# OrangeSodahub/ORV

Measured on AMD Instinct MI355X. Metric: denoise-steps/sec, higher is better.
Workload: dtype bf16; 1 GPU; configs[1]: CogVideoX-2B singleview 320x480x17f (latents [B,5,32,40,60], S=3226), DDIM 50-step schedule, guidance 1.0, trajectory-conditioned; batch_per_gpu=4, num_layers=30, parallelism=replica x1 (no collective), valid=True

## Files before the change

orv_amd/csrc/gemm_d8.hip:

```cpp
#include "gemm_common.hpp"
#include <type_traits>

namespace {
using namespace orv_gemm;

__device__ __forceinline__ void d8_unpack8(const uint4 u, float (&f)[8]) {
    f[0] = bf2f(u.x & 0xffff); f[1] = bf2f(u.x >> 16); f[2] = bf2f(u.y & 0xffff); f[3] = bf2f(u.y >> 16);
    f[4] = bf2f(u.z & 0xffff); f[5] = bf2f(u.z >> 16); f[6] = bf2f(u.w & 0xffff); f[7] = bf2f(u.w >> 16);
}
__device__ __forceinline__ uint4 d8_pack8(const float (&f)[8]) {
    return make_uint4(pack2bf(f[0], f[1]), pack2bf(f[2], f[3]), pack2bf(f[4], f[5]), pack2bf(f[6], f[7]));
}
__device__ __forceinline__ float d8_sum_quad(float v) {
    v += __uint_as_float(__builtin_amdgcn_update_dpp(0, __float_as_uint(v), 0xB1, 0xF, 0xF, true));
    v += __uint_as_float(__builtin_amdgcn_update_dpp(0, __float_as_uint(v), 0x4E, 0xF, 0xF, true));
    return v;
}
__device__ __forceinline__ float d8_shl4(float v) {
    return __uint_as_float(__builtin_amdgcn_update_dpp(0, __float_as_uint(v), 0x104, 0xF, 0xF, true));
}
__device__ __forceinline__ float d8_shr4(float v) {
    return __uint_as_float(__builtin_amdgcn_update_dpp(0, __float_as_uint(v), 0x114, 0xF, 0xF, true));
}
__device__ __forceinline__ unsigned long long d8_uniform64(unsigned long long u) {
    const unsigned lo = __builtin_amdgcn_readfirstlane((unsigned)u), hi = __builtin_amdgcn_readfirstlane((unsigned)(u >> 32));
    return ((unsigned long long)hi << 32) | lo;
}

__device__ __forceinline__ void d8_glds_v(const void* gsrc, const char* lds_dst) {
    const unsigned d = __builtin_amdgcn_readfirstlane((unsigned)(uintptr_t)(const __attribute__((address_space(3))) char*)lds_dst);
    asm volatile("s_mov_b32 m0, %1\n\ts_nop 0\n\tglobal_load_lds_dwordx4 %0, off" :: "v"(gsrc), "s"(d) : "memory", "m0");
}
__device__ __forceinline__ void d8_issue_rows(const GemmArgs& p, const int row0, const int colg, const int lane, const char* slab) {
#pragma unroll
    for (int j = 0; j < 4; ++j) {
        const int mc = min(row0 + 8 * j + (lane >> 3), p.M - 1);
        long rr = mc;
        if (p.r_mod > 0) rr = mc % p.r_mod;
        else if (p.c_rows > 0) rr = (long)(mc / p.c_rows) * p.c_bstride + p.c_off + mc % p.c_rows;
        d8_glds_v(p.R + rr * p.ldr + colg + 8 * (lane & 7), slab + j * 1024);
    }
}
template <int BN, int EPI>
constexpr bool d8_rlds() {
#ifdef ORV_D8_RLDS
    return BN <= 192 && (EPI == 2 || EPI == 3);
#else
    return false;
#endif
}

template <int BN, int EPI, int RB = 2>
__device__ __forceinline__ void d8_epilogue(const GemmArgs& p, f32x4 (&acc)[RB][BN / 16], const int row0, const int col0, const int lane,
                                            char* const scr, const char* const rslab = nullptr) {
    constexpr int NG = BN / 64;
    constexpr bool RLDS = d8_rlds<BN, EPI>();
    const int g = lane >> 4, r16 = lane & 15;
    const int c = lane & 7, rr8 = lane >> 3;
    int woff[4];
#pragma unroll
    for (int blk = 0; blk < 4; ++blk) {
        const int L = 8 * (blk >> 1) + 2 * g + (blk & 1);
        woff[blk] = r16 * 256 + ((L ^ (r16 & 7)) << 4);
    }
    const int roff0 = rr8 * 256 + (((2 * c) ^ rr8) << 4), roff1 = rr8 * 256 + (((2 * c + 1) ^ rr8) << 4);

    constexpr bool GATH = EPI == 2 || EPI == 3;
    using row_t = std::conditional_t<GATH && BN == 256, int, long>;
    row_t orow[RB][2];
    bool valid[RB][2];
#pragma unroll
    for (int rb = 0; rb < RB; ++rb)
#pragma unroll
        for (int j = 0; j < 2; ++j) {
            const int m = row0 + rb * 16 + 8 * j + rr8;
            valid[rb][j] = m < p.M;
            const int mc = min(m, p.M - 1);
            orow[rb][j] = mc;
            if (p.c_rows > 0) orow[rb][j] = (row_t)((long)(mc / p.c_rows) * p.c_bstride + p.c_off + mc % p.c_rows);
        }
    const float *gate_a = nullptr, *gate_b = nullptr;
    int gseg = 0;
    bool in_a[RB][2];
#pragma unroll
    for (int rb = 0; rb < RB; ++rb) in_a[rb][0] = in_a[rb][1] = true;
    if (EPI == 2 && p.gate) {
        const int mf = __builtin_amdgcn_readfirstlane(row0);
        long of = min(mf, p.M - 1), ol = min(mf + 16 * RB - 1, p.M - 1);
        if (p.c_rows > 0) {
            of = (long)(of / p.c_rows) * p.c_bstride + p.c_off + of % p.c_rows;
            ol = (long)(ol / p.c_rows) * p.c_bstride + p.c_off + ol % p.c_rows;
        }
        const int bf_ = (int)(of / p.seq), bl_ = (int)(ol / p.seq);
        const int gf_ = orv_group_of((int)(of % p.seq), p.n_text, p.per_group);
        const int gl_ = orv_group_of((int)(ol % p.seq), p.n_text, p.per_group);
        gate_a = p.gate + bf_ * p.gate_b + gf_ * p.gate_g;
        gseg = 1;
        if (bf_ != bl_ || gf_ != gl_) {
            gate_b = p.gate + bl_ * p.gate_b + gl_ * p.gate_g;
            const int ea_ = gf_ == 0 ? p.n_text : (p.per_group > 0 ? p.n_text + gf_ * p.per_group : p.seq);
            const long end_a = (long)bf_ * p.seq + min(ea_, p.seq);
            const long start_b = (long)bl_ * p.seq + (gl_ == 0 ? 0 : p.n_text + (gl_ - 1) * max(p.per_group, 0));
            bool other = false;
#pragma unroll
            for (int rb = 0; rb < RB; ++rb)
#pragma unroll
                for (int j = 0; j < 2; ++j) {
                    in_a[rb][j] = orow[rb][j] < end_a;
                    other = other || !(in_a[rb][j] || orow[rb][j] >= start_b);
                }
            gseg = (BN == 256 || __builtin_amdgcn_ballot_w64(other) != 0) ? 3 : 2;
        }
    }
    uint4 r8[RB][2];
    auto load_row = [&](int cg, int rb, int j) {
        long rr = orow[rb][j];
        if (p.r_mod > 0) rr = min(row0 + rb * 16 + 8 * j + rr8, p.M - 1) % p.r_mod;
        return *(const uint4*)(p.R + rr * p.ldr + col0 + 64 * cg + 8 * c);
    };
    auto take_rows = [&](int cg, uint4 (&dst)[RB][2]) {
        asm volatile("s_waitcnt vmcnt(0)" ::: "memory");
        __builtin_amdgcn_sched_barrier(0);
#pragma unroll
        for (int rb = 0; rb < RB; ++rb)
#pragma unroll
            for (int j = 0; j < 2; ++j) dst[rb][j] = *(const uint4*)(rslab + (rb * 16 + 8 * j + rr8) * 128 + c * 16);
        if (cg + 1 < NG) {
            asm volatile("s_waitcnt lgkmcnt(0)" ::: "memory");
            __builtin_amdgcn_sched_barrier(0);
            d8_issue_rows(p, row0, col0 + 64 * (cg + 1), lane, rslab);
        }
    };
    if (RLDS) {
        take_rows(0, r8);
    } else if (GATH) {
#pragma unroll
        for (int rb = 0; rb < RB; ++rb)
#pragma unroll
            for (int j = 0; j < 2; ++j) r8[rb][j] = load_row(0, rb, j);
    }
    const int bp = c << 5;
    uint32_t bsrc[NG];
    float gsrc_a[NG], gsrc_b[NG];
#pragma unroll
    for (int cg = 0; cg < NG; ++cg) { bsrc[cg] = 0; gsrc_a[cg] = gsrc_b[cg] = 1.f; }
    if constexpr (GATH) {
        if (p.bias) {
#pragma unroll
            for (int cg = 0; cg < NG; ++cg) bsrc[cg] = p.bias[col0 + 64 * cg + lane];
        }
        if (gseg == 1 || gseg == 2) {
#pragma unroll
            for (int cg = 0; cg < NG; ++cg) gsrc_a[cg] = gate_a[col0 + 64 * cg + lane];
        }
        if (gseg == 2) {
#pragma unroll
            for (int cg = 0; cg < NG; ++cg) gsrc_b[cg] = gate_b[col0 + 64 * cg + lane];
        }
    }
    auto spread8 = [&](uint32_t src, uint32_t (&o)[8]) {
        asm volatile("ds_bpermute_b32 %0, %8, %9\n\tds_bpermute_b32 %1, %8, %9 offset:4\n\tds_bpermute_b32 %2, %8, %9 offset:8\n\t"
                     "ds_bpermute_b32 %3, %8, %9 offset:12\n\tds_bpermute_b32 %4, %8, %9 offset:16\n\tds_bpermute_b32 %5, %8, %9 offset:20\n\t"
                     "ds_bpermute_b32 %6, %8, %9 offset:24\n\tds_bpermute_b32 %7, %8, %9 offset:28\n\ts_waitcnt lgkmcnt(0)"
                     : "=&v"(o[0]), "=&v"(o[1]), "=&v"(o[2]), "=&v"(o[3]), "=&v"(o[4]), "=&v"(o[5]), "=&v"(o[6]), "=&v"(o[7])
                     : "v"(bp), "v"(src));
    };

#pragma unroll
    for (int cg = 0; cg < NG; ++cg) {
        const int col8 = col0 + 64 * cg + 8 * c;
        if (RLDS && cg > 0) take_rows(cg, r8);
        float b8[8];
#pragma unroll
        for (int e = 0; e < 8; ++e) b8[e] = 0.f;
        if (p.bias) {
            if constexpr (GATH) {
                uint32_t o[8];
                spread8(bsrc[cg], o);
#pragma unroll
                for (int e = 0; e < 8; ++e) b8[e] = bf2f((bf16_t)o[e]);
            } else {
                d8_unpack8(*(const uint4*)(p.bias + col8), b8);
            }
        }
        float ga[8], be[8];
        int region = 2;
        float post = 1.f;
        if constexpr (EPI == 4) {
            region = __builtin_amdgcn_readfirstlane((col0 + 64 * cg) / (p.qn_heads * 64));
            const bf16_t* gam = region == 0 ? p.qn_gq : p.qn_gk;
            const bf16_t* bet = region == 0 ? p.qn_bq : p.qn_bk;
            post = region == 0 ? p.qn_premul : 1.f;
#pragma unroll
            for (int e = 0; e < 8; ++e) { ga[e] = 1.f; be[e] = 0.f; }
            if (region < 2 && gam) d8_unpack8(*(const uint4*)(gam + 8 * c), ga);
            if (region < 2 && bet) d8_unpack8(*(const uint4*)(bet + 8 * c), be);
        }
        float g8[8];
#pragma unroll
        for (int e = 0; e < 8; ++e) g8[e] = 1.f;
        if (gseg == 1 || gseg == 2) {
            uint32_t o[8];
            spread8(__float_as_uint(gsrc_a[cg]), o);
#pragma unroll
            for (int e = 0; e < 8; ++e) g8[e] = __uint_as_float(o[e]);
        }

#pragma unroll
        for (int rb = 0; rb < RB; ++rb) {
#pragma unroll
            for (int blk = 0; blk < 4; ++blk) *(f32x4*)(scr + woff[blk]) = acc[rb][4 * cg + blk];
            float v[2][8];
            auto read_v = [&](int j) {
                const f32x4 lo = *(const f32x4*)(scr + j * 2048 + roff0), hi = *(const f32x4*)(scr + j * 2048 + roff1);
                v[j][0] = lo[0]; v[j][1] = lo[1]; v[j][2] = lo[2]; v[j][3] = lo[3];
                v[j][4] = hi[0]; v[j][5] = hi[1]; v[j][6] = hi[2]; v[j][7] = hi[3];
            };
            if constexpr (!GATH) { read_v(0); read_v(1); }
#pragma unroll
            for (int j = 0; j < 2; ++j) {
                if constexpr (GATH) {
                    asm volatile("" ::: "memory");
                    read_v(j);
                }
                float (&w)[8] = v[j];
                uint4 rcur;
                if constexpr (GATH) {
                    rcur = r8[rb][j];
                    if (!RLDS && cg + 1 < NG) r8[rb][j] = load_row(cg + 1, rb, j);
                }
#pragma unroll
                for (int e = 0; e < 8; ++e) w[e] += b8[e];
                bf16_t* crow = p.C + orow[rb][j] * p.ldc + col8;
                if (p.Y && valid[rb][j]) *(uint4*)(p.Y + orow[rb][j] * p.ldy + col8) = d8_pack8(w);
                if constexpr (EPI == 4) {
                    if (region < 2) {
                        float hi[8];
#pragma unroll
                        for (int e = 0; e < 8; ++e) hi[e] = d8_shl4(w[e]);
                        float s = 0.f;
#pragma unroll
                        for (int e = 0; e < 8; ++e) s += w[e];
#pragma unroll
                        for (int e = 0; e < 8; ++e) s += hi[e];
                        s = d8_sum_quad(s);
                        const float s_up = d8_shr4(s);
                        const float mean = (c < 4 ? s : s_up) * (1.f / 64.f);
                        float sq = 0.f;
#pragma unroll
                        for (int e = 0; e < 8; ++e) { w[e] -= mean; sq = qkln_sq(w[e], sq); }
#pragma unroll
                        for (int e = 0; e < 8; ++e) { hi[e] -= mean; sq = qkln_sq(hi[e], sq); }
                        sq = d8_sum_quad(sq);
                        const float sq_up = d8_shr4(sq);
                        const float rstd = rsqrtf((c < 4 ? sq : sq_up) * (1.f / 64.f) + p.qn_eps);
#pragma unroll
                        for (int e = 0; e < 8; ++e) w[e] = qkln_affine(w[e], rstd, ga[e], be[e], post);
                    }
                }
                if (EPI == 1) {
#pragma unroll
                    for (int e = 0; e < 8; ++e) w[e] = gelu_tanh(w[e]);
                }
                if (EPI == 2) {
                    float rv[8], gg[8];
                    d8_unpack8(rcur, rv);
#pragma unroll
                    for (int e = 0; e < 8; ++e) gg[e] = g8[e];
                    if (gseg == 2) {
                        uint32_t o[8];
                        spread8(__float_as_uint(gsrc_b[cg]), o);
#pragma unroll
                        for (int e = 0; e < 8; ++e) gg[e] = in_a[rb][j] ? g8[e] : __uint_as_float(o[e]);
                    }
                    if (gseg == 3 && j == 0) {
                        f32x4 q[2][2];
#pragma unroll
                        for (int jj = 0; jj < 2; ++jj) {
                            const unsigned o_ = (unsigned)orow[rb][jj];
                            const int bidx = (int)(o_ / (unsigned)p.seq), sq_ = (int)(o_ - (unsigned)bidx * (unsigned)p.seq);
                            const float* grow = p.gate + bidx * p.gate_b + orv_group_of(sq_, p.n_text, p.per_group) * p.gate_g;
                            q[jj][0] = *(const f32x4*)(grow + col8);
                            q[jj][1] = *(const f32x4*)(grow + col8 + 4);
                        }
                        asm volatile("" : "+v"(q[0][0]), "+v"(q[0][1]), "+v"(q[1][0]), "+v"(q[1][1]));
#pragma unroll
                        for (int e = 0; e < 8; ++e) { gg[e] = q[0][e >> 2][e & 3]; g8[e] = q[1][e >> 2][e & 3]; }
                    }
#pragma unroll
                    for (int e = 0; e < 8; ++e) w[e] = rv[e] + gg[e] * w[e];
                }
                if (EPI == 3) {
                    float rv[8];
                    d8_unpack8(rcur, rv);
#pragma unroll
                    for (int e = 0; e < 8; ++e) w[e] *= gelu_tanh_grad(rv[e]);
                }
                if (valid[rb][j]) *(uint4*)crow = d8_pack8(w);
            }
        }
    }
}

template <int BN, int EPI, int RB = 2>
__device__ __forceinline__ void d8_epilogue_packed(const GemmArgs& p, f32x4 (&acc)[RB][BN / 16], const int row0, const int col0, const int lane) {
    const int g = lane >> 4;
    const long nblk = p.ldc / 32;
#pragma unroll
    for (int P = 0; P < BN / 32; ++P) {
        float b8[8];
#pragma unroll
        for (int e = 0; e < 8; ++e) b8[e] = 0.f;
        if (p.bias) d8_unpack8(*(const uint4*)(p.bias + col0 + 32 * P + 8 * g), b8);
#pragma unroll
        for (int rb = 0; rb < RB; ++rb) {
            float v[8];
#pragma unroll
            for (int e = 0; e < 8; ++e) v[e] = acc[rb][2 * P + (e >> 2)][e & 3] + b8[e];
            if (EPI == 1) {
#pragma unroll
                for (int e = 0; e < 8; ++e) v[e] = gelu_tanh(v[e]);
            }
            char* blk = (char*)p.C + (((long)(row0 / 16 + rb) * nblk + (col0 / 32 + P)) << 10);
            *(uint4*)(blk + lane * 16) = d8_pack8(v);
        }
    }
}

template <int BN, int EPI, int RB, int BM>
__device__ __forceinline__ void d8_body(const GemmArgs& p, char* const smem) {
    static_assert(BM == 256 || BM == 192, "tile rows");
    static_assert(!(d8_rlds<BN, EPI>() && BM != 256), "the residual slab path is written for 32-row waves");
    constexpr int NA = 2 * RB;
    constexpr int NCB = BN / 16;
#ifndef ORV_D8_CBP256
#define ORV_D8_CBP256 2
#endif
#ifndef ORV_D8_CBP192
#define ORV_D8_CBP192 3
#endif
    constexpr int CBP = BN == 256 ? ORV_D8_CBP256 : (BN == 192 ? ORV_D8_CBP192 : 2);
    constexpr int NPH = NCB / CBP;
    constexpr int BUFSZ = BN * 128;
    constexpr int ND = BN / 64;
    constexpr int SCR = 4 * BUFSZ;
    const int lane = threadIdx.x & 63;
    const int wave = __builtin_amdgcn_readfirstlane(threadIdx.x >> 6);
    const int wrb = (BM == 256 || RB == 2) ? 2 * wave : 8 + (wave - 4);
    const int ntiles = p.tiles_m * p.tiles_n;
    const int nk = p.K / BK;

    const int dr = lane >> 3;
    const unsigned voffW = (unsigned)(((long)(8 * (dr >> 2) + (dr & 3)) * p.ldw + (((lane & 7) ^ (dr & 6)) << 3)) * 2);
    unsigned long long wb[ND], wbn[ND];
    int kW = 0, tW = blockIdx.x;
    const unsigned lds0 = (unsigned)(uintptr_t)(const __attribute__((address_space(3))) char*)smem;
#define D8_SETUP_W(DST, TILE)                                                                                        \
    {                                                                                                                \
        int tm_, tn_;                                                                                                \
        tile_of_index(p, min((TILE), ntiles - 1), ntiles, tm_, tn_);                                                 \
        _Pragma("unroll") for (int j = 0; j < ND; ++j) {                                                             \
            const int q_ = wave * ND + j, cb_ = q_ >> 1;                                                             \
            const int wrow_ = tn_ * BN + 32 * (cb_ >> 1) + 16 * (q_ & 1) + 4 * (cb_ & 1);                            \
            DST[j] = d8_uniform64((unsigned long long)(uintptr_t)p.W + (unsigned long long)wrow_ * p.ldw * 2);       \
        }                                                                                                            \
    }
#define D8_WRAP_W()                                                                                                  \
    {                                                                                                                \
        const bool w_ = ++kW == nk;                                                                                  \
        kW = w_ ? 0 : kW;                                                                                            \
        tW += w_ ? (int)gridDim.x : 0;                                                                               \
        _Pragma("unroll") for (int j = 0; j < ND; ++j) wb[j] = w_ ? wbn[j] : wb[j];                                  \
    }
#ifdef ORV_D8_ABL_NODMA
#define D8_DMA1(OFF, SB, LDS) asm volatile("" :: "v"(OFF), "s"(SB), "s"(LDS));
#else
#define D8_DMA1(OFF, SB, LDS) asm volatile("s_mov_b32 m0, %2\n\ts_nop 0\n\tglobal_load_lds_dwordx4 %0, %1" :: "v"(OFF), "s"(SB), "s"(LDS) : "memory", "m0");
#endif
#define D8_ISSUE_W(BUFI)                                                                                             \
    {                                                                                                                \
        _Pragma("unroll") for (int j = 0; j < ND; ++j) {                                                             \
            const unsigned long long sb_ = wb[j] + (unsigned long long)kW * 128;                                     \
            const unsigned ld_ = lds0 + (BUFI) * BUFSZ + (wave * ND + j) * 1024;                                     \
            D8_DMA1(voffW, sb_, ld_)                                                                                 \
        }                                                                                                            \
        D8_WRAP_W()                                                                                                  \
    }
    D8_SETUP_W(wb, tW)
    D8_SETUP_W(wbn, tW + (int)gridDim.x)

    unsigned voffA[2];
    const unsigned long long rowblk = (unsigned long long)p.K * 32;
    unsigned long long ab, abn;
    int kA = 0, tA = blockIdx.x;
    voffA[0] = (unsigned)lane * 16;
    voffA[1] = (unsigned)lane * 16 + (unsigned)rowblk;
#define D8_SETUP_A(DST, TILE)                                                                                        \
    {                                                                                                                \
        int tm_, tn_;                                                                                                \
        tile_of_index(p, min((TILE), ntiles - 1), ntiles, tm_, tn_);                                                 \
        DST = d8_uniform64((unsigned long long)(uintptr_t)p.A + (unsigned long long)(tm_ * (BM / 16) + wrb) * rowblk); \
    }
#define D8_WRAP_A()                                                                                                  \
    {                                                                                                                \
        const bool w_ = ++kA == nk;                                                                                  \
        kA = w_ ? 0 : kA;                                                                                            \
        tA += w_ ? (int)gridDim.x : 0;                                                                               \
        ab = w_ ? abn : ab;                                                                                          \
    }
#ifdef ORV_D8_ABL_NOA
#define D8_LOADA(DST, OFF, SB, IMM) asm volatile("" : "=v"(DST) : "v"(OFF), "s"(SB));
#else
#define D8_LOADA(DST, OFF, SB, IMM) asm volatile("global_load_dwordx4 %0, %1, %2 offset:" #IMM : "=v"(DST) : "v"(OFF), "s"(SB) : "memory");
#endif
#define D8_ISSUE_A(SET)                                                                                              \
    {                                                                                                                \
        const unsigned long long sa_ = ab + (unsigned long long)kA * 2048;                                           \
        D8_LOADA(SET[0], voffA[0], sa_, 0) D8_LOADA(SET[1], voffA[0], sa_, 1024)                                     \
        if constexpr (RB == 2) { D8_LOADA(SET[NA - 2], voffA[1], sa_, 0) D8_LOADA(SET[NA - 1], voffA[1], sa_, 1024) } \
        D8_WRAP_A()                                                                                                  \
    }
    D8_SETUP_A(ab, tA)
    D8_SETUP_A(abn, tA + (int)gridDim.x)

    const int fro = ((lane & 15) >> 3) * 1024 + (lane & 7) * 128 + (((lane >> 4) ^ (lane & 6)) << 4);
    const char* const rd0 = smem + fro;
    const char* const rd1 = smem + (fro ^ 64);

    f32x4 acc[RB][NCB];
#pragma unroll
    for (int a = 0; a < RB; ++a)
#pragma unroll
        for (int b = 0; b < NCB; ++b) acc[a][b] = f32x4{0.f, 0.f, 0.f, 0.f};
    bf16x8 a0[NA], a1[NA], a2[NA];
    bf16x8 fx[CBP][2];

#define D8_FENCE() __builtin_amdgcn_sched_barrier(0);
#ifdef ORV_D8_ABL_NOREAD
#define D8_READ1(T, KH, BOFF, PH) asm volatile("" : "+v"(fx[T][KH]));
#elif defined(ORV_D8_ABL_READ2)
#define D8_READ1(T, KH, BOFF, PH)                                                                                    \
    { fx[T][KH] = *(const bf16x8*)(((KH) ? rd1 : rd0) + (BOFF) + ((PH) * CBP + (T)) * 2048);                         \
      bf16x8 dummy_ = *(const volatile bf16x8*)(((KH) ? rd0 : rd1) + (BOFF) + ((PH) * CBP + (T)) * 2048); asm volatile("" :: "v"(dummy_)); }
#else
#define D8_READ1(T, KH, BOFF, PH) fx[T][KH] = *(const bf16x8*)(((KH) ? rd1 : rd0) + (BOFF) + ((PH) * CBP + (T)) * 2048);
#endif
#ifdef ORV_D8_ABL_NOMFMA
#define D8_MFMA1(T, KH, AS, PH)                                                                                      \
    _Pragma("unroll") for (int rb = 0; rb < RB; ++rb) asm volatile("" : "+v"(acc[rb][(PH) * CBP + (T)]) : "v"(fx[T][KH]), "v"(AS[rb * 2 + (KH)]));
#else
#define D8_MFMA1(T, KH, AS, PH)                                                                                      \
    _Pragma("unroll") for (int rb = 0; rb < RB; ++rb)                                                                \
        acc[rb][(PH) * CBP + (T)] = __builtin_amdgcn_mfma_f32_16x16x32_bf16(fx[T][KH], AS[rb * 2 + (KH)], acc[rb][(PH) * CBP + (T)], 0, 0, 0);
#endif
#define D8_SLOT(S, ANEW, DBUF)                                                                                       \
    if ((S) < ND) {                                                                                                  \
        const unsigned long long sb_ = wb[(S) < ND ? (S) : 0] + (unsigned long long)kW * 128;                        \
        const unsigned ld_ = lds0 + (DBUF) * BUFSZ + (wave * ND + (S)) * 1024;                                       \
        D8_DMA1(voffW, sb_, ld_)                                                                                     \
        if ((S) == ND - 1) D8_WRAP_W()                                                                               \
    } else if ((S) < ND + NA) {                                                                                      \
        const unsigned long long sa_ = ab + (unsigned long long)kA * 2048;                                           \
        if ((S) == ND) D8_LOADA(ANEW[0], voffA[0], sa_, 0)                                                           \
        if ((S) == ND + 1) D8_LOADA(ANEW[1], voffA[0], sa_, 1024)                                                    \
        if constexpr (RB == 2) {                                                                                     \
            if ((S) == ND + 2) D8_LOADA(ANEW[NA - 2], voffA[1], sa_, 0)                                              \
            if ((S) == ND + 3) D8_LOADA(ANEW[NA - 1], voffA[1], sa_, 1024)                                           \
        }                                                                                                            \
        if ((S) == ND + NA - 1) D8_WRAP_A()                                                                          \
    }
#define D8_STEP_SLOT(PH, S, ANEW, DBUF)                                                                              \
    _Pragma("unroll") for (int i_ = 0; i_ < ND + NA; ++i_)                                                           \
        if ((PH) * 2 * CBP + (S) == ((2 * i_ + 1) * 2 * NCB) / (2 * (ND + NA))) { D8_SLOT(i_, ANEW, DBUF) }
#define D8_PHASE(RBUF, RPH, ACUR, ANEW, PH, DBUF)                                                                    \
    _Pragma("unroll") for (int s_ = 0; s_ < 2 * CBP; ++s_) {                                                         \
        D8_MFMA1(s_ % CBP, s_ / CBP, ACUR, PH) D8_FENCE()                                                            \
        D8_READ1(s_ % CBP, s_ / CBP, RBUF, RPH) D8_FENCE()                                                           \
        D8_STEP_SLOT(PH, s_, ANEW, DBUF) D8_FENCE()                                                                  \
    }
#ifdef ORV_D8_ABL_NOWAIT
#define D8_WAIT(ACUR)                                                                                                \
    if constexpr (RB == 2) asm volatile("" : "+v"(ACUR[0]), "+v"(ACUR[1]), "+v"(ACUR[2]), "+v"(ACUR[3]));            \
    else asm volatile("" : "+v"(ACUR[0]), "+v"(ACUR[1]));
#else
#define D8_WAIT(ACUR)                                                                                                \
    if constexpr (RB == 2) asm volatile("s_waitcnt vmcnt(%4)" : "+v"(ACUR[0]), "+v"(ACUR[1]), "+v"(ACUR[2]), "+v"(ACUR[3]) : "n"(ND + NA) : "memory"); \
    else asm volatile("s_waitcnt vmcnt(%2)" : "+v"(ACUR[0]), "+v"(ACUR[1]) : "n"(ND + NA) : "memory");
#endif
#ifdef ORV_D8_ABL_LNA
    const float lna_rs = p.qn_eps == 12345.f ? 2.f : 1.f, lna_nm = p.qn_eps == 12345.f ? 1.f : 0.f;
    float lna_g[8], lna_s[8];
    _Pragma("unroll") for (int e_ = 0; e_ < 8; ++e_) { lna_g[e_] = p.qn_premul == 54321.f ? 3.f + e_ : 1.f; lna_s[e_] = p.qn_premul == 54321.f ? 1.f : 0.f; }
#define D8_LNA(ACUR)                                                                                                 \
    _Pragma("unroll") for (int i_ = 0; i_ < NA; ++i_) {                                                              \
        union { bf16x8 v; uint32_t u[4]; } c_; c_.v = ACUR[i_];                                                      \
        _Pragma("unroll") for (int w_ = 0; w_ < 4; ++w_) {                                                           \
            const float lo_ = __builtin_fmaf(__builtin_fmaf(bf2f(c_.u[w_] & 0xffff), lna_rs, lna_nm), lna_g[2 * w_], lna_s[2 * w_]);          \
            const float hi_ = __builtin_fmaf(__builtin_fmaf(bf2f(c_.u[w_] >> 16), lna_rs, lna_nm), lna_g[2 * w_ + 1], lna_s[2 * w_ + 1]);     \
            c_.u[w_] = pack2bf(lo_, hi_);                                                                            \
        }                                                                                                            \
        ACUR[i_] = c_.v;                                                                                             \
    }
#else
#define D8_LNA(ACUR)
#endif
#define D8_KTILE(ACUR, ANEW)                                                                                         \
    {                                                                                                                \
        D8_WAIT(ACUR)                                                                                                \
        D8_LNA(ACUR)                                                                                                 \
        D8_FENCE() __builtin_amdgcn_s_barrier(); D8_FENCE()                                                          \
        const int cur_ = bufc * BUFSZ, nxt_ = ((bufc + 1) & 3) * BUFSZ, dbuf_ = (bufc + 3) & 3;                      \
        _Pragma("unroll") for (int pp_ = 0; pp_ < NPH; ++pp_) {                                                      \
            D8_PHASE((pp_ + 1 < NPH ? cur_ : nxt_), (pp_ + 1) % NPH, ACUR, ANEW, pp_, dbuf_)                         \
        }                                                                                                            \
        bufc = (bufc + 1) & 3;                                                                                       \
    }

    int bufc = 0;
    D8_ISSUE_W(0)
    D8_ISSUE_W(1) D8_ISSUE_A(a0)
    D8_ISSUE_W(2) D8_ISSUE_A(a1)
    asm volatile("s_waitcnt vmcnt(%0)" :: "n"(2 * (ND + NA)) : "memory");
    D8_FENCE() __builtin_amdgcn_s_barrier(); D8_FENCE()
    _Pragma("unroll") for (int s_ = 0; s_ < 2 * CBP; ++s_) { D8_READ1(s_ % CBP, s_ / CBP, 0, 0) }
    D8_FENCE()

    for (int tile = blockIdx.x; tile < ntiles; tile += gridDim.x) {
        D8_SETUP_W(wbn, tW + (int)gridDim.x)
        D8_SETUP_A(abn, tA + (int)gridDim.x)
        for (int kt = 0; kt < nk; kt += 3) {
            if (d8_rlds<BN, EPI>() && kt + 3 >= nk) {
                int tm_, tn_;
                tile_of_index(p, tile, ntiles, tm_, tn_);
                d8_issue_rows(p, tm_ * BM + wrb * 16, tn_ * BN, lane, smem + SCR + 8 * 4096 + wave * 4096);
            }
            D8_KTILE(a0, a2)
            D8_KTILE(a1, a0)
            D8_KTILE(a2, a1)
        }
        int tm, tn;
        tile_of_index(p, tile, ntiles, tm, tn);
#ifdef ORV_D8_ABL_NOEPI
        _Pragma("unroll") for (int a_ = 0; a_ < RB; ++a_)
            _Pragma("unroll") for (int b_ = 0; b_ < NCB; ++b_) asm volatile("" :: "v"(acc[a_][b_]));
#else
        if ((EPI == 0 || EPI == 1) && p.c_packed) d8_epilogue_packed<BN, EPI, RB>(p, acc, tm * BM + wrb * 16, tn * BN, lane);
        else d8_epilogue<BN, EPI, RB>(p, acc, tm * BM + wrb * 16, tn * BN, lane, smem + SCR + wave * 4096, smem + SCR + 8 * 4096 + wave * 4096);
        if constexpr (BN == 256 && (EPI == 2 || EPI == 3)) {
            D8_FENCE()
            _Pragma("unroll") for (int s_ = 0; s_ < 2 * CBP; ++s_) { D8_READ1(s_ % CBP, s_ / CBP, bufc * BUFSZ, 0) }
            D8_FENCE()
        }
#endif
#pragma unroll
        for (int a = 0; a < RB; ++a)
#pragma unroll
            for (int b = 0; b < NCB; ++b) acc[a][b] = f32x4{0.f, 0.f, 0.f, 0.f};
    }
    asm volatile("s_waitcnt vmcnt(0)" ::: "memory");
    asm volatile("" :: "v"(a0[0]), "v"(a1[0]), "v"(a2[0]), "v"(fx[0][0]));
}

template <int BN, int EPI>
__global__ __launch_bounds__(512) void gemm_d8_kernel(const GemmArgs p) {
    extern __shared__ __attribute__((aligned(16))) char smem[];
    d8_body<BN, EPI, 2, 256>(p, smem);
}
template <int BN, int EPI>
__global__ __launch_bounds__(512) void gemm_d8r192_kernel(const GemmArgs p) {
    extern __shared__ __attribute__((aligned(16))) char smem[];
    if (__builtin_amdgcn_readfirstlane(threadIdx.x >> 6) < 4) d8_body<BN, EPI, 2, 192>(p, smem);
    else d8_body<BN, EPI, 1, 192>(p, smem);
}

template <int BN, int EPI, int BM>
int launch_d8_one(const GemmArgs& a, hipStream_t st) {
    constexpr int smem = 4 * BN * 128 + 8 * 4096 + (d8_rlds<BN, EPI>() ? 8 * 4096 : 0);
    void (*kern)(const GemmArgs);
    if constexpr (BM == 256) kern = gemm_d8_kernel<BN, EPI>;
    else kern = gemm_d8r192_kernel<BN, EPI>;
    static bool attr_done = false;
    if (!attr_done) {
        (void)hipFuncSetAttribute((const void*)kern, hipFuncAttributeMaxDynamicSharedMemorySize, smem);
        attr_done = true;
    }
    int grid = min(a.tiles_m * a.tiles_n, orv_num_cus());
    if (a.grid_cap > 0) grid = min(grid, a.grid_cap);
    hipLaunchKernelGGL(kern, dim3(grid), dim3(512), smem, st, a);
    return orv_check_launch("orv_gemm_bf16");
}

}

namespace orv_gemm {
int launch_d8(const GemmArgs& a, int bn, int epi, hipStream_t st, int bm) {
    if (!a.a_packed || (long)a.N * a.ldw * 2 >= (1L << 32) || a.K % 192 != 0 || a.lda != a.K) {
        orv_set_error("orv_gemm_bf16: the d8 kernel needs a packed A (a_packed, lda == K), K %% 192 == 0 and W below 4 GiB (lda=%ld N=%d ldw=%ld K=%d)",
                      a.lda, a.N, a.ldw, a.K);
        return ORV_EINVAL;
    }
    if (a.c_packed && (epi > 1 || a.ldc != a.N || a.c_rows > 0 || a.Y)) {
        orv_set_error("orv_gemm_bf16: packed C needs epilogue 0 / 1, ldc == N, no row map, no Y");
        return ORV_EINVAL;
    }
    if (epi == 2 || epi == 3) {
        const long last = a.c_rows > 0 ? (long)((a.M - 1) / a.c_rows) * a.c_bstride + a.c_off + a.c_rows - 1 : (long)a.M - 1;
        if (last >= (1L << 31) || (epi == 2 && a.gate && a.seq <= 0)) {
            orv_set_error("orv_gemm_bf16: the row-operand epilogues need output rows below 2^31 and seq > 0 (last row %ld, seq=%d)", last, a.seq);
            return ORV_EINVAL;
        }
    }
    if (bm == 192) {
        if ((long)a.tiles_m * 192 > ((long)a.M + 255) / 256 * 256) {
            orv_set_error("orv_gemm_bf16: 192-row d8 tiles would read past the packed row slots (M=%d)", a.M);
            return ORV_EINVAL;
        }
        if (bn == 128) {
            switch (epi) {
                case 0: return launch_d8_one<128, 0, 192>(a, st);
                case 1: return launch_d8_one<128, 1, 192>(a, st);
                case 2: return launch_d8_one<128, 2, 192>(a, st);
                case 4: return launch_d8_one<128, 4, 192>(a, st);
            }
        } else if (bn == 192) {
            switch (epi) {
                case 0: return launch_d8_one<192, 0, 192>(a, st);
                case 1: return launch_d8_one<192, 1, 192>(a, st);
                case 2: return launch_d8_one<192, 2, 192>(a, st);
                case 4: return launch_d8_one<192, 4, 192>(a, st);
            }
        }
        orv_set_error("orv_gemm_bf16: no 192-row d8 kernel for BN=%d epilogue %d", bn, epi);
        return ORV_EINVAL;
    }
    if (bn == 256) {
        switch (epi) {
            case 0: return launch_d8_one<256, 0, 256>(a, st);
            case 1: return launch_d8_one<256, 1, 256>(a, st);
            case 2: return launch_d8_one<256, 2, 256>(a, st);
            case 3: return launch_d8_one<256, 3, 256>(a, st);
            case 4: return launch_d8_one<256, 4, 256>(a, st);
        }
    } else if (bn == 128) {
        switch (epi) {
            case 0: return launch_d8_one<128, 0, 256>(a, st);
            case 1: return launch_d8_one<128, 1, 256>(a, st);
            case 2: return launch_d8_one<128, 2, 256>(a, st);
            case 4: return launch_d8_one<128, 4, 256>(a, st);
        }
    } else if (bn == 192) {
        switch (epi) {
            case 0: return launch_d8_one<192, 0, 256>(a, st);
            case 1: return launch_d8_one<192, 1, 256>(a, st);
            case 2: return launch_d8_one<192, 2, 256>(a, st);
            case 3: return launch_d8_one<192, 3, 256>(a, st);
            case 4: return launch_d8_one<192, 4, 256>(a, st);
        }
    }
    orv_set_error("orv_gemm_bf16: no d8 kernel for BN=%d epilogue %d", bn, epi);
    return ORV_EINVAL;
}
}

namespace {
__global__ __launch_bounds__(256) void pack_rows16_kernel(const bf16_t* src, long ld, uint4* dst, int M, int K, long pieces) {
    const long d = (long)blockIdx.x * 256 + threadIdx.x;
    if (d >= pieces) return;
    const long blk = d >> 6;
    const int l = (int)(d & 63), kb = K / 32;
    const long row = (blk / kb) * 16 + (l & 15);
    const int k = (int)(blk % kb) * 32 + (l >> 4) * 8;
    dst[d] = row < M ? *(const uint4*)(src + row * ld + k) : make_uint4(0, 0, 0, 0);
}
__global__ __launch_bounds__(256) void unpack_rows16_kernel(const uint4* src, bf16_t* dst, long ld, int M, int K, long pieces) {
    const long d = (long)blockIdx.x * 256 + threadIdx.x;
    if (d >= pieces) return;
    const int kc = K / 8;
    const long row = d / kc;
    const int c = (int)(d % kc);
    const long blk = (row >> 4) * (K / 32) + (c >> 2);
    *(uint4*)(dst + row * ld + c * 8) = src[blk * 64 + (c & 3) * 16 + (row & 15)];
}
}
extern "C" long orv_packed_rows(long rows) { return (rows + 255) / 256 * 256; }
extern "C" int orv_pack_rows16(const void* src, long ld_src, void* dst, int M, int K, void* stream) {
    ORV_REQUIRE(src && dst && M > 0 && K > 0 && K % 32 == 0 && ld_src % 8 == 0, "orv_pack_rows16: bad arguments (M=%d K=%d ld=%ld)", M, K, ld_src);
    const long pieces = orv_packed_rows(M) * (K / 8);
    hipLaunchKernelGGL(pack_rows16_kernel, dim3((unsigned)((pieces + 255) / 256)), dim3(256), 0, (hipStream_t)stream, (const bf16_t*)src, ld_src,
                       (uint4*)dst, M, K, pieces);
    return orv_check_launch("orv_pack_rows16");
}
extern "C" int orv_unpack_rows16(const void* src, void* dst, long ld_dst, int M, int K, void* stream) {
    ORV_REQUIRE(src && dst && M > 0 && K > 0 && K % 32 == 0 && ld_dst % 8 == 0, "orv_unpack_rows16: bad arguments (M=%d K=%d ld=%ld)", M, K, ld_dst);
    const long pieces = (long)M * (K / 8);
    hipLaunchKernelGGL(unpack_rows16_kernel, dim3((unsigned)((pieces + 255) / 256)), dim3(256), 0, (hipStream_t)stream, (const uint4*)src,
                       (bf16_t*)dst, ld_dst, M, K, pieces);
    return orv_check_launch("orv_unpack_rows16");
}
```

Baseline: 104.1 steps/s (clips x denoise steps per second).

## Prefetch epilogue bias, gate and residual rows into LDS during last K tile

Replaces the ifdef-gated residual slab path with an always-on staged path for BN<=192 gated/residual epilogues. During the final K-tile iteration, per-tile bias, gate rows and the first residual row chunk are issued into per-wave LDS with global_load_lds, overlapping the MMA loop. The epilogue then reads them from LDS instead of using ds_bpermute spreads and direct global loads. Row mapping and gate segment setup are hoisted before the K loop. This adds LDS use per block and an alignment requirement on gate rows, and adjusts vmcnt waits.

New measurement: 104.1 steps/s (clips x denoise steps per second). About the same (-0.0%).

```diff
diff --git a/orv_amd/csrc/gemm_d8.hip b/orv_amd/csrc/gemm_d8.hip
--- a/orv_amd/csrc/gemm_d8.hip
+++ b/orv_amd/csrc/gemm_d8.hip
@@ -31,30 +31,85 @@
     const unsigned d = __builtin_amdgcn_readfirstlane((unsigned)(uintptr_t)(const __attribute__((address_space(3))) char*)lds_dst);
     asm volatile("s_mov_b32 m0, %1\n\ts_nop 0\n\tglobal_load_lds_dwordx4 %0, off" :: "v"(gsrc), "s"(d) : "memory", "m0");
 }
-__device__ __forceinline__ void d8_issue_rows(const GemmArgs& p, const int row0, const int colg, const int lane, const char* slab) {
-#pragma unroll
-    for (int j = 0; j < 4; ++j) {
-        const int mc = min(row0 + 8 * j + (lane >> 3), p.M - 1);
-        long rr = mc;
-        if (p.r_mod > 0) rr = mc % p.r_mod;
-        else if (p.c_rows > 0) rr = (long)(mc / p.c_rows) * p.c_bstride + p.c_off + mc % p.c_rows;
-        d8_glds_v(p.R + rr * p.ldr + colg + 8 * (lane & 7), slab + j * 1024);
-    }
+__device__ __forceinline__ void d8_glds_s(const unsigned voff, const void* sbase, const char* lds_dst) {
+    const unsigned d = __builtin_amdgcn_readfirstlane((unsigned)(uintptr_t)(const __attribute__((address_space(3))) char*)lds_dst);
+    const unsigned long long sb = (unsigned long long)(uintptr_t)sbase;
+    asm volatile("s_mov_b32 m0, %2\n\ts_nop 0\n\tglobal_load_lds_dwordx4 %0, %1" :: "v"(voff), "s"(sb), "s"(d) : "memory", "m0");
 }
 template <int BN, int EPI>
-constexpr bool d8_rlds() {
-#ifdef ORV_D8_RLDS
-    return BN <= 192 && (EPI == 2 || EPI == 3);
-#else
-    return false;
-#endif
+constexpr bool d8_staged() { return BN <= 192 && (EPI == 2 || EPI == 3); }
+constexpr int D8_VEC = 3072;
+
+struct D8Gate {
+    const float *a, *b;
+    long end_a, start_b;
+    int seg;
+};
+template <int RB>
+__device__ __forceinline__ D8Gate d8_gate_rows(const GemmArgs& p, const int row0) {
+    D8Gate G{nullptr, nullptr, 0, 0, 0};
+    const int mf = __builtin_amdgcn_readfirstlane(row0);
+    long of = min(mf, p.M - 1), ol = min(mf + 16 * RB - 1, p.M - 1);
+    if (p.c_rows > 0) {
+        of = (long)(of / p.c_rows) * p.c_bstride + p.c_off + of % p.c_rows;
+        ol = (long)(ol / p.c_rows) * p.c_bstride + p.c_off + ol % p.c_rows;
+    }
+    const int bf_ = (int)(of / p.seq), bl_ = (int)(ol / p.seq);
+    const int gf_ = orv_group_of((int)(of % p.seq), p.n_text, p.per_group);
+    const int gl_ = orv_group_of((int)(ol % p.seq), p.n_text, p.per_group);
+    G.a = p.gate + bf_ * p.gate_b + gf_ * p.gate_g;
+    G.seg = 1;
+    if (bf_ != bl_ || gf_ != gl_) {
+        G.b = p.gate + bl_ * p.gate_b + gl_ * p.gate_g;
+        const int ea_ = gf_ == 0 ? p.n_text : (p.per_group > 0 ? p.n_text + gf_ * p.per_group : p.seq);
+        G.end_a = (long)bf_ * p.seq + min(ea_, p.seq);
+        G.start_b = (long)bl_ * p.seq + (gl_ == 0 ? 0 : p.n_text + (gl_ - 1) * max(p.per_group, 0));
+        G.seg = 2;
+    }
+    return G;
+}
+
+template <int RB>
+struct D8Tail {
+    long orow[RB][2];
+    const bf16_t* rsrc[RB][2];
+    D8Gate gate;
+};
+template <int BN_, int EPI, int RB>
+__device__ __forceinline__ void d8_tail_setup(const GemmArgs& p, const int row0, const int col0, const int lane, D8Tail<RB>& t) {
+#pragma unroll
+    for (int rb = 0; rb < RB; ++rb)
+#pragma unroll
+        for (int j = 0; j < 2; ++j) {
+            const int mc = min(row0 + rb * 16 + 8 * j + (lane >> 3), p.M - 1);
+            long o = mc;
+            if (p.c_rows > 0) o = (long)(mc / p.c_rows) * p.c_bstride + p.c_off + mc % p.c_rows;
+            t.orow[rb][j] = o;
+            const long rr = p.r_mod > 0 ? (long)(mc % p.r_mod) : o;
+            t.rsrc[rb][j] = p.R + rr * p.ldr + col0 + 8 * (lane & 7);
+        }
+    t.gate = D8Gate{nullptr, nullptr, 0, 0, 0};
+    if (EPI == 2 && p.gate) t.gate = d8_gate_rows<RB>(p, row0);
+}
+template <int BN, int RB>
+__device__ __forceinline__ void d8_tail_issue(const GemmArgs& p, const D8Tail<RB>& t, const int col0, const int lane, const char* scr,
+                                              const char* vec) {
+    asm volatile("s_waitcnt lgkmcnt(0)" ::: "memory");
+    const unsigned vb = (unsigned)min(lane, BN / 8 - 1) * 16, vg = (unsigned)min(lane, BN / 4 - 1) * 16;
+    if (p.bias) d8_glds_s(vb, p.bias + col0, vec);
+    if (t.gate.seg >= 1) d8_glds_s(vg, t.gate.a + col0, vec + 1024);
+    if (t.gate.seg == 2) d8_glds_s(vg, t.gate.b + col0, vec + 2048);
+#pragma unroll
+    for (int rb = 0; rb < RB; ++rb)
+#pragma unroll
+        for (int j = 0; j < 2; ++j) d8_glds_v(t.rsrc[rb][j], scr + (2 * rb + j) * 1024);
 }
 
 template <int BN, int EPI, int RB = 2>
 __device__ __forceinline__ void d8_epilogue(const GemmArgs& p, f32x4 (&acc)[RB][BN / 16], const int row0, const int col0, const int lane,
-                                            char* const scr, const char* const rslab = nullptr) {
+                                            char* const scr, const char* const vec = nullptr, const D8Tail<RB>* const tail = nullptr) {
     constexpr int NG = BN / 64;
-    constexpr bool RLDS = d8_rlds<BN, EPI>();
+    constexpr bool STG = d8_staged<BN, EPI>();
     const int g = lane >> 4, r16 = lane & 15;
     const int c = lane & 7, rr8 = lane >> 3;
     int woff[4];
@@ -76,8 +131,12 @@
             const int m = row0 + rb * 16 + 8 * j + rr8;
             valid[rb][j] = m < p.M;
             const int mc = min(m, p.M - 1);
-            orow[rb][j] = mc;
-            if (p.c_rows > 0) orow[rb][j] = (row_t)((long)(mc / p.c_rows) * p.c_bstride + p.c_off + mc % p.c_rows);
+            if constexpr (STG) {
+                orow[rb][j] = tail->orow[rb][j];
+            } else {
+                orow[rb][j] = mc;
+                if (p.c_rows > 0) orow[rb][j] = (row_t)((long)(mc / p.c_rows) * p.c_bstride + p.c_off + mc % p.c_rows);
+            }
         }
     const float *gate_a = nullptr, *gate_b = nullptr;
     int gseg = 0;
@@ -85,29 +144,20 @@
 #pragma unroll
     for (int rb = 0; rb < RB; ++rb) in_a[rb][0] = in_a[rb][1] = true;
     if (EPI == 2 && p.gate) {
-        const int mf = __builtin_amdgcn_readfirstlane(row0);
-        long of = min(mf, p.M - 1), ol = min(mf + 16 * RB - 1, p.M - 1);
-        if (p.c_rows > 0) {
-            of = (long)(of / p.c_rows) * p.c_bstride + p.c_off + of % p.c_rows;
-            ol = (long)(ol / p.c_rows) * p.c_bstride + p.c_off + ol % p.c_rows;
-        }
-        const int bf_ = (int)(of / p.seq), bl_ = (int)(ol / p.seq);
-        const int gf_ = orv_group_of((int)(of % p.seq), p.n_text, p.per_group);
-        const int gl_ = orv_group_of((int)(ol % p.seq), p.n_text, p.per_group);
-        gate_a = p.gate + bf_ * p.gate_b + gf_ * p.gate_g;
+        D8Gate G;
+        if constexpr (STG) G = tail->gate;
+        else G = d8_gate_rows<RB>(p, row0);
+        gate_a = G.a;
         gseg = 1;
-        if (bf_ != bl_ || gf_ != gl_) {
-            gate_b = p.gate + bl_ * p.gate_b + gl_ * p.gate_g;
-            const int ea_ = gf_ == 0 ? p.n_text : (p.per_group > 0 ? p.n_text + gf_ * p.per_group : p.seq);
-            const long end_a = (long)bf_ * p.seq + min(ea_, p.seq);
-            const long start_b = (long)bl_ * p.seq + (gl_ == 0 ? 0 : p.n_text + (gl_ - 1) * max(p.per_group, 0));
+        if (G.seg == 2) {
+            gate_b = G.b;
             bool other = false;
 #pragma unroll
             for (int rb = 0; rb < RB; ++rb)
 #pragma unroll
                 for (int j = 0; j < 2; ++j) {
-                    in_a[rb][j] = orow[rb][j] < end_a;
-                    other = other || !(in_a[rb][j] || orow[rb][j] >= start_b);
+                    in_a[rb][j] = orow[rb][j] < G.end_a;
+                    other = other || !(in_a[rb][j] || orow[rb][j] >= G.start_b);
                 }
             gseg = (BN == 256 || __builtin_amdgcn_ballot_w64(other) != 0) ? 3 : 2;
         }
@@ -118,21 +168,11 @@
         if (p.r_mod > 0) rr = min(row0 + rb * 16 + 8 * j + rr8, p.M - 1) % p.r_mod;
         return *(const uint4*)(p.R + rr * p.ldr + col0 + 64 * cg + 8 * c);
     };
-    auto take_rows = [&](int cg, uint4 (&dst)[RB][2]) {
-        asm volatile("s_waitcnt vmcnt(0)" ::: "memory");
-        __builtin_amdgcn_sched_barrier(0);
+    if constexpr (STG) {
 #pragma unroll
         for (int rb = 0; rb < RB; ++rb)
 #pragma unroll
-            for (int j = 0; j < 2; ++j) dst[rb][j] = *(const uint4*)(rslab + (rb * 16 + 8 * j + rr8) * 128 + c * 16);
-        if (cg + 1 < NG) {
-            asm volatile("s_waitcnt lgkmcnt(0)" ::: "memory");
-            __builtin_amdgcn_sched_barrier(0);
-            d8_issue_rows(p, row0, col0 + 64 * (cg + 1), lane, rslab);
-        }
-    };
-    if (RLDS) {
-        take_rows(0, r8);
+            for (int j = 0; j < 2; ++j) r8[rb][j] = *(const uint4*)(scr + (2 * rb + j) * 1024 + lane * 16);
     } else if (GATH) {
 #pragma unroll
         for (int rb = 0; rb < RB; ++rb)
@@ -144,7 +184,7 @@
     float gsrc_a[NG], gsrc_b[NG];
 #pragma unroll
     for (int cg = 0; cg < NG; ++cg) { bsrc[cg] = 0; gsrc_a[cg] = gsrc_b[cg] = 1.f; }
-    if constexpr (GATH) {
+    if constexpr (GATH && !STG) {
         if (p.bias) {
 #pragma unroll
             for (int cg = 0; cg < NG; ++cg) bsrc[cg] = p.bias[col0 + 64 * cg + lane];
@@ -169,12 +209,13 @@
 #pragma unroll
     for (int cg = 0; cg < NG; ++cg) {
         const int col8 = col0 + 64 * cg + 8 * c;
-        if (RLDS && cg > 0) take_rows(cg, r8);
         float b8[8];
 #pragma unroll
         for (int e = 0; e < 8; ++e) b8[e] = 0.f;
         if (p.bias) {
-            if constexpr (GATH) {
+            if constexpr (STG) {
+                d8_unpack8(*(const uint4*)(vec + (64 * cg + 8 * c) * 2), b8);
+            } else if constexpr (GATH) {
                 uint32_t o[8];
                 spread8(bsrc[cg], o);
 #pragma unroll
@@ -200,10 +241,16 @@
 #pragma unroll
         for (int e = 0; e < 8; ++e) g8[e] = 1.f;
         if (gseg == 1 || gseg == 2) {
-            uint32_t o[8];
-            spread8(__float_as_uint(gsrc_a[cg]), o);
-#pragma unroll
-            for (int e = 0; e < 8; ++e) g8[e] = __uint_as_float(o[e]);
+            if constexpr (STG) {
+                const f32x4 lo = *(const f32x4*)(vec + 1024 + (64 * cg + 8 * c) * 4), hi = *(const f32x4*)(vec + 1024 + (64 * cg + 8 * c) * 4 + 16);
+#pragma unroll
+                for (int e = 0; e < 4; ++e) { g8[e] = lo[e]; g8[4 + e] = hi[e]; }
+            } else {
+                uint32_t o[8];
+                spread8(__float_as_uint(gsrc_a[cg]), o);
+#pragma unroll
+                for (int e = 0; e < 8; ++e) g8[e] = __uint_as_float(o[e]);
+            }
         }
 
 #pragma unroll
@@ -227,7 +274,7 @@
                 uint4 rcur;
                 if constexpr (GATH) {
                     rcur = r8[rb][j];
-                    if (!RLDS && cg + 1 < NG) r8[rb][j] = load_row(cg + 1, rb, j);
+                    if (cg + 1 < NG) r8[rb][j] = load_row(cg + 1, rb, j);
                 }
 #pragma unroll
                 for (int e = 0; e < 8; ++e) w[e] += b8[e];
@@ -264,14 +311,27 @@
                 }
                 if (EPI == 2) {
                     float rv[8], gg[8];
+                    if constexpr (STG && (BN == 128 || RB == 1)) {
+                        typedef uint32_t u32x4_ __attribute__((ext_vector_type(4)));
+                        u32x4_ t_ = {rcur.x, rcur.y, rcur.z, rcur.w};
+                        asm volatile("" : "+v"(t_));
+                        rcur = make_uint4(t_.x, t_.y, t_.z, t_.w);
+                    }
                     d8_unpack8(rcur, rv);
 #pragma unroll
                     for (int e = 0; e < 8; ++e) gg[e] = g8[e];
                     if (gseg == 2) {
-                        uint32_t o[8];
-                        spread8(__float_as_uint(gsrc_b[cg]), o);
-#pragma unroll
-                        for (int e = 0; e < 8; ++e) gg[e] = in_a[rb][j] ? g8[e] : __uint_as_float(o[e]);
+                        if constexpr (STG) {
+                            const f32x4 lo = *(const f32x4*)(vec + 2048 + (64 * cg + 8 * c) * 4);
+                            const f32x4 hi = *(const f32x4*)(vec + 2048 + (64 * cg + 8 * c) * 4 + 16);
+#pragma unroll
+                            for (int e = 0; e < 4; ++e) { gg[e] = in_a[rb][j] ? g8[e] : lo[e]; gg[4 + e] = in_a[rb][j] ? g8[4 + e] : hi[e]; }
+                        } else {
+                            uint32_t o[8];
+                            spread8(__float_as_uint(gsrc_b[cg]), o);
+#pragma unroll
+                            for (int e = 0; e < 8; ++e) gg[e] = in_a[rb][j] ? g8[e] : __uint_as_float(o[e]);
+                        }
                     }
                     if (gseg == 3 && j == 0) {
                         f32x4 q[2][2];
@@ -330,7 +390,7 @@
 template <int BN, int EPI, int RB, int BM>
 __device__ __forceinline__ void d8_body(const GemmArgs& p, char* const smem) {
     static_assert(BM == 256 || BM == 192, "tile rows");
-    static_assert(!(d8_rlds<BN, EPI>() && BM != 256), "the residual slab path is written for 32-row waves");
+    constexpr bool STG = d8_staged<BN, EPI>();
     constexpr int NA = 2 * RB;
     constexpr int NCB = BN / 16;
 #ifndef ORV_D8_CBP256
@@ -504,11 +564,22 @@
 #else
 #define D8_LNA(ACUR)
 #endif
-#define D8_KTILE(ACUR, ANEW)                                                                                         \
+#define D8_KTILE(ACUR, ANEW, Q)                                                                                      \
     {                                                                                                                \
-        D8_WAIT(ACUR)                                                                                                \
+        if constexpr (STG && (Q) == 1) {                                                                             \
+            if (tail_) asm volatile("s_waitcnt vmcnt(%0)" :: "n"(ND + NA + 2 * RB) : "memory");                      \
+            else asm volatile("s_waitcnt vmcnt(%0)" :: "n"(ND + NA) : "memory");                                     \
+            if constexpr (RB == 2) asm volatile("" : "+v"(ACUR[0]), "+v"(ACUR[1]), "+v"(ACUR[2]), "+v"(ACUR[3]));    \
+            else asm volatile("" : "+v"(ACUR[0]), "+v"(ACUR[1]));                                                    \
+        } else {                                                                                                     \
+            D8_WAIT(ACUR)                                                                                            \
+        }                                                                                                            \
         D8_LNA(ACUR)                                                                                                 \
         D8_FENCE() __builtin_amdgcn_s_barrier(); D8_FENCE()                                                          \
+        if constexpr (STG && (Q) == 0) {                                                                             \
+            if (tail_) d8_tail_issue<BN, RB>(p, tl, tn * BN, lane, smem + SCR + wave * 4096, smem + SCR + 8 * 4096 + wave * D8_VEC); \
+            D8_FENCE()                                                                                               \
+        }                                                                                                            \
         const int cur_ = bufc * BUFSZ, nxt_ = ((bufc + 1) & 3) * BUFSZ, dbuf_ = (bufc + 3) & 3;                      \
         _Pragma("unroll") for (int pp_ = 0; pp_ < NPH; ++pp_) {                                                      \
             D8_PHASE((pp_ + 1 < NPH ? cur_ : nxt_), (pp_ + 1) % NPH, ACUR, ANEW, pp_, dbuf_)                         \
@@ -528,24 +599,25 @@
     for (int tile = blockIdx.x; tile < ntiles; tile += gridDim.x) {
         D8_SETUP_W(wbn, tW + (int)gridDim.x)
         D8_SETUP_A(abn, tA + (int)gridDim.x)
+        int tm = 0, tn = 0;
+        D8Tail<RB> tl;
+        if constexpr (STG) {
+            tile_of_index(p, tile, ntiles, tm, tn);
+            d8_tail_setup<BN, EPI, RB>(p, tm * BM + wrb * 16, tn * BN, lane, tl);
+        }
         for (int kt = 0; kt < nk; kt += 3) {
-            if (d8_rlds<BN, EPI>() && kt + 3 >= nk) {
-                int tm_, tn_;
-                tile_of_index(p, tile, ntiles, tm_, tn_);
-                d8_issue_rows(p, tm_ * BM + wrb * 16, tn_ * BN, lane, smem + SCR + 8 * 4096 + wave * 4096);
-            }
-            D8_KTILE(a0, a2)
-            D8_KTILE(a1, a0)
-            D8_KTILE(a2, a1)
-        }
-        int tm, tn;
-        tile_of_index(p, tile, ntiles, tm, tn);
+            const bool tail_ = kt + 3 >= nk;
+            D8_KTILE(a0, a2, 0)
+            D8_KTILE(a1, a0, 1)
+            D8_KTILE(a2, a1, 2)
+        }
+        if constexpr (!STG) tile_of_index(p, tile, ntiles, tm, tn);
 #ifdef ORV_D8_ABL_NOEPI
         _Pragma("unroll") for (int a_ = 0; a_ < RB; ++a_)
             _Pragma("unroll") for (int b_ = 0; b_ < NCB; ++b_) asm volatile("" :: "v"(acc[a_][b_]));
 #else
         if ((EPI == 0 || EPI == 1) && p.c_packed) d8_epilogue_packed<BN, EPI, RB>(p, acc, tm * BM + wrb * 16, tn * BN, lane);
-        else d8_epilogue<BN, EPI, RB>(p, acc, tm * BM + wrb * 16, tn * BN, lane, smem + SCR + wave * 4096, smem + SCR + 8 * 4096 + wave * 4096);
+        else d8_epilogue<BN, EPI, RB>(p, acc, tm * BM + wrb * 16, tn * BN, lane, smem + SCR + wave * 4096, smem + SCR + 8 * 4096 + wave * D8_VEC, &tl);
         if constexpr (BN == 256 && (EPI == 2 || EPI == 3)) {
             D8_FENCE()
             _Pragma("unroll") for (int s_ = 0; s_ < 2 * CBP; ++s_) { D8_READ1(s_ % CBP, s_ / CBP, bufc * BUFSZ, 0) }
@@ -575,7 +647,7 @@
 
 template <int BN, int EPI, int BM>
 int launch_d8_one(const GemmArgs& a, hipStream_t st) {
-    constexpr int smem = 4 * BN * 128 + 8 * 4096 + (d8_rlds<BN, EPI>() ? 8 * 4096 : 0);
+    constexpr int smem = 4 * BN * 128 + 8 * 4096 + (d8_staged<BN, EPI>() ? 8 * D8_VEC : 0);
     void (*kern)(const GemmArgs);
     if constexpr (BM == 256) kern = gemm_d8_kernel<BN, EPI>;
     else kern = gemm_d8r192_kernel<BN, EPI>;
@@ -607,6 +679,10 @@
         const long last = a.c_rows > 0 ? (long)((a.M - 1) / a.c_rows) * a.c_bstride + a.c_off + a.c_rows - 1 : (long)a.M - 1;
         if (last >= (1L << 31) || (epi == 2 && a.gate && a.seq <= 0)) {
             orv_set_error("orv_gemm_bf16: the row-operand epilogues need output rows below 2^31 and seq > 0 (last row %ld, seq=%d)", last, a.seq);
+            return ORV_EINVAL;
+        }
+        if (epi == 2 && a.gate && ((uintptr_t)a.gate % 16 != 0 || a.gate_b % 4 != 0 || a.gate_g % 4 != 0)) {
+            orv_set_error("orv_gemm_bf16: the gated epilogue needs 16-byte aligned gate rows (gate_b=%ld gate_g=%ld)", a.gate_b, a.gate_g);
             return ORV_EINVAL;
         }
     }
```
